# microsoft/NOTSOFAR1-Challenge

Hardware: AMD Instinct MI355X
Metric: CSS real-time-factor (sep. audio sec/wall sec) on 7-ch 16 kHz (higher is better)
Workload: dtype f32 (float32 operands on v_mfma_f32_32x32x2_f32 in every Linear layer, attention product and transform: the reference's own operand precision; MVDR covariance / solve f64)

## Files before the change

### notsofar1-challenge_amd/csrc/api_core.hip

```cpp
#include "api_ctx.hpp"

thread_local std::string g_create_error;

int fail(css_ctx* h, int code, const std::string& msg) {
    if (h) h->err = msg;
    else g_create_error = msg;
    return code;
}

int ensure(css_ctx* h, DevBuf& b, size_t bytes, bool zero) {
    if (bytes <= b.cap) return CSS_OK;
    if (b.p && h->queued) HIPCHK(h, hipDeviceSynchronize());
    if (b.p) HIPCHK(h, hipFree(b.p));
    b.p = nullptr;
    b.cap = 0;
    HIPCHK(h, hipMalloc(&b.p, bytes));
    b.cap = bytes;
    if (zero) HIPCHK(h, hipMemsetAsync(b.p, 0, bytes, h->stream));
    return CSS_OK;
}

int64_t bind_weights(const CssModelDesc& d, const float* base, Weights* w) {
    const int64_t D = d.attention_dim, FF = d.linear_units, Kp = round_up(d.in_features, 32);
    const int64_t dk = D / d.attention_heads, ks = d.kernel_size;
// ... 585 lines not shown
    if (!h || lanes < 1 || lanes > css_ctx::MAX_LANES) return fail(h, CSS_ERR_INVALID_ARG, "lanes must be in [1, 4]");
    h->lanes = lanes;
    return CSS_OK;
}

int css_get_lanes(css_handle_t h) { return h ? h->lanes : (int)CSS_ERR_INVALID_ARG; }

int css_set_tuning(css_handle_t h, int which, int value) {
    if (!h || which < 0 || which >= CSS_TUNE_COUNT || value < 0 || (value > 16 && which != CSS_TUNE_SPLIT_BATCH_ROWS && which != CSS_TUNE_F32_LANE_ROWS))
        return fail(h, CSS_ERR_INVALID_ARG, "unknown tuning option / value");
    h->tune[which] = value;
    return CSS_OK;
}

int css_set_range_fallback(css_handle_t h, int enable) {
    if (!h) return CSS_ERR_INVALID_ARG;
    h->range_fallback = enable != 0;
    return CSS_OK;
}

int css_range_status(css_handle_t h, int64_t* fallbacks, int32_t* last_hit) {
    if (!h) return CSS_ERR_INVALID_ARG;
    if (fallbacks) *fallbacks = h->range_fallbacks;
    if (last_hit) *last_hit = h->range_last;
    return CSS_OK;
}

int css_check_range(css_handle_t h) {
    int rc = check_session(h);
    if (rc) return rc;
    HIPCHK(h, hipSetDevice(h->device));
    HIPCHK(h, hipMemcpyAsync(h->range_flag_host, h->range_flag_dev, sizeof(unsigned int), hipMemcpyDeviceToHost, h->stream));
    HIPCHK(h, hipStreamSynchronize(h->stream));
    if (*h->range_flag_host && h->split)
        return fail(h, CSS_ERR_RANGE, "an operand of a Linear layer left the split-f16 range (|x| > 65504): use CSS_LINEAR_EXACT_F32");
    return CSS_OK;
}

int css_linear_host(css_handle_t h, const float* x, const float* w, const float* bias, int32_t M, int32_t N, int32_t K,
                    int32_t kernel, int32_t layout, float* y) {
    CSS_DRAIN(h);
    if (!h || !x || !w || !y || M < 1 || N < 1 || K < 32 || K % 32) return fail(h, CSS_ERR_INVALID_ARG, "bad argument (K must be a multiple of 32)");
    if (kernel < 0 || kernel > 2) return fail(h, CSS_ERR_INVALID_ARG, "kernel must be 0 (split, weights direct), 1 (split, LDS staged) or 2 (exact float32)");
    HIPCHK(h, hipSetDevice(h->device));
    const int Np = (N + 31) / 32 * 32;
    const size_t xf = (size_t)M * K, wf = (size_t)Np * K, yf = (size_t)M * N;
    int rc;
    if ((rc = ensure(h, h->stage, (2 * xf + 2 * wf + yf + (size_t)N + 256) * sizeof(float))) != CSS_OK) return rc;
    float* xd = (float*)h->stage.p;
    float* xs = xd + (xf + 15) / 16 * 16;
    float* wd = xs + (xf + 15) / 16 * 16;
    float* ws = wd + (wf + 15) / 16 * 16;
    float* yd = ws + (wf + 15) / 16 * 16;
    float* bd = yd + (yf + 15) / 16 * 16;
    HIPCHK(h, hipMemcpyAsync(xd, x, xf * sizeof(float), hipMemcpyHostToDevice, h->stream));
    HIPCHK(h, hipMemcpyAsync(wd, w, (size_t)N * K * sizeof(float), hipMemcpyHostToDevice, h->stream));
    if (bias) HIPCHK(h, hipMemcpyAsync(bd, bias, (size_t)N * sizeof(float), hipMemcpyHostToDevice, h->stream));
    GemmArgs g = linear(xd, K, wd, K, bias ? bd : nullptr, yd, N, M, N, K, ACT_NONE);
    if (kernel != 2) {
        launch_split_convert(xd, K, xs, M, K, K, h->stream);
        if (kernel == 0) launch_split_convert_tiled(wd, K, ws, N, K, h->stream);
        else launch_split_convert(wd, K, ws, N, K, K, h->stream);
        g.A = xs; g.B = ws; g.split_in = 1; g.b_tiled = kernel == 0;
        if (kernel == 0) g.tile_rows = layout; else g.layout = layout;
    } else {
        g.layout = layout;
    }
    launch_gemm(g, h->stream);
    HIPCHK(h, hipMemcpyAsync(y, yd, yf * sizeof(float), hipMemcpyDeviceToHost, h->stream));
    HIPCHK(h, hipStreamSynchronize(h->stream));
    HIPCHK(h, hipGetLastError());
    return CSS_OK;
}

int css_gemm_host(css_handle_t h, const CssGemmDesc* d, const float* a, const float* b, const float* bias, const float* residual,
                  float* c) {
    CSS_DRAIN(h);
    if (!h) return CSS_ERR_INVALID_ARG;
    auto bad = [&](const char* what) { return fail(h, CSS_ERR_INVALID_ARG, std::string("css_gemm_host: ") + what); };
    if (!d || !a || !b || !c) return bad("null argument");
    const int64_t cap = (int64_t)1 << 28;
    const int M = d->M, N = d->N, K = d->K, batch = d->batch, kernel = d->kernel;
    if (kernel < 0 || kernel > 2) return bad("kernel must be 0 (split, weights direct), 1 (split, LDS staged) or 2 (exact float32)");
    if (M < 1 || N < 1 || batch < 1 || K < 32 || K % 32 || M > (1 << 22) || N > (1 << 22) || K > (1 << 16) || batch > 1024)
        return bad("M, N, batch >= 1 and K a multiple of 32");
    if (d->lda < K || d->ldb < K || d->lda % 4 || d->ldb % 4 || d->lda > cap || d->ldb > cap) return bad("lda, ldb: multiples of 4, at least K");
    if (d->act < ACT_NONE || d->act > ACT_SIGMOID) return bad("act must be 0, 1 or 2");
    if (d->bias < 0 || d->bias > 2 || (d->bias != 0) != (bias != nullptr)) return bad("bias: 0 with NULL, 1 or 2 with an array");
    if (d->residual < 0 || d->residual > 2 || (d->residual == 1) != (residual != nullptr)) return bad("residual: 1 with an array, 0 or 2 with NULL");
    if (!(std::fabs(d->alpha) <= 3.0e38f)) return bad("alpha must be finite");
    if (d->a_off < 0 || d->c_off < 0 || d->r_off < 0 || d->a_off > 1024 || d->c_off > (1 << 20) || d->r_off > 1024) return bad("offsets");
    const bool tr = d->c_transposed != 0, has_res = d->residual != 0;
    const int rows_c = tr ? N : M, cols_c = tr ? M : N;
    if (d->ldc < cols_c || d->ldc > cap) return bad("ldc is shorter than a row of C");
    const int64_t ldr = d->residual == 2 ? d->ldc : d->ldr;
    if (d->residual == 1 && (ldr < N || ldr > cap)) return bad("ldr is shorter than a row of the residual");
    if (d->residual == 2 && batch != 1) return bad("the in-place residual takes batch 1");
    const int64_t extA = (int64_t)(M - 1) * d->lda + K, extB = (int64_t)(N - 1) * d->ldb + K;
    const int64_t extC = (int64_t)(rows_c - 1) * d->ldc + cols_c, extR = (int64_t)(M - 1) * ldr + N;
    const int64_t sA = batch > 1 ? d->strideA : 0, sB = batch > 1 ? d->strideB : 0, sC = batch > 1 ? d->strideC : 0;
    if (sA < 0 || sB < 0 || sA > cap || sB > cap || sC > cap || (sA && sA < extA) || (sB && sB < extB)) return bad("strideA, strideB: 0 or at least one matrix");
    if (batch > 1 && sC < extC) return bad("batch entries of C overlap");
    if (d->a_floats > cap || d->b_floats > cap || d->c_floats > cap || d->r_floats > cap) return bad("an array of more than 2^28 floats");
    if (d->a_floats < d->a_off + (batch - 1) * sA + extA) return bad("a is shorter than its description");
    if (d->b_floats < (batch - 1) * sB + extB) return bad("b is shorter than its description");
    if (d->c_floats < d->c_off + (batch - 1) * sC + extC) return bad("c is shorter than its description");
    if (d->residual == 1 && d->r_floats < d->r_off + extR) return bad("residual is shorter than its description");
    if (d->split_out < 0 || d->split_out % 32 || d->split_out > N || (d->split_out && kernel == 2)) return bad("split_out: a multiple of 32 up to N, kernels 0 and 1");
    if (tr && (kernel != 0 || has_res || d->split_out || d->bias == 2)) return bad("c_transposed: kernel 0, column bias and activation only");
    if (kernel == 0 && (batch != 1 || N % 32)) return bad("kernel 0 takes batch 1 and whole 32-column weight tiles");
    if (kernel == 0 && !tr && (d->c_off % 4 || d->ldc % 4)) return bad("kernel 0 writes 16-byte pieces: c_off and ldc must be multiples of 4");
    if (d->b_frag32 && (kernel != 2 || batch != 1 || N % 32)) return bad("b_frag32: kernel 2, batch 1, N a multiple of 32");
    const int lay = d->layout, tile = d->tile_rows;
    const bool lay_ok = kernel == 0 ? lay == 0
                                    : (lay == 0 || lay == 8 || lay == 4 || lay == 64 || (kernel == 2 && (lay == 1 || lay == 2 || (lay >= 11 && lay <= 14))));
    const bool tile_ok = kernel == 0 ? (tile == 0 || tile == 32 || tile == 64 || tile == 96 || tile == 128 || tile == 4 || tile == 65) : tile == 0;
    if (!lay_ok || !tile_ok) return bad("layout / tile_rows: not a tile layout of this kernel");

    HIPCHK(h, hipSetDevice(h->device));
    auto pad = [](int64_t n) { return (size_t)((n + 63) / 64 * 64); };
    const int nA = sA ? batch : 1, nB = sB ? batch : 1;
    const int Np = (N + 31) / 32 * 32;
    const size_t f_a = pad(d->a_floats), f_b = pad(d->b_floats), f_c = pad(d->c_floats), f_r = pad(d->residual == 1 ? d->r_floats : 0);
    const size_t f_as = kernel != 2 ? pad((int64_t)nA * M * K) : 0, f_bs = kernel == 0 ? pad((int64_t)Np * K) : kernel == 1 ? pad((int64_t)nB * N * K) : 0;
    const size_t f_bf = d->b_frag32 ? pad((int64_t)N * K) : 0, f_bias = pad(d->bias == 2 ? M : N);
    int rc;
    if ((rc = ensure(h, h->stage, (f_a + f_b + f_c + f_r + f_as + f_bs + f_bf + f_bias) * sizeof(float))) != CSS_OK) return rc;
    float* ad = (float*)h->stage.p;
    float* bd = ad + f_a;
    float* cd = bd + f_b;
    float* rd = cd + f_c;
    float* as = rd + f_r;
    float* bs = as + f_as;
    float* bf = bs + f_bs;
    float* biasd = bf + f_bf;
    HIPCHK(h, hipMemcpyAsync(ad, a, (size_t)d->a_floats * sizeof(float), hipMemcpyHostToDevice, h->stream));
    HIPCHK(h, hipMemcpyAsync(bd, b, (size_t)d->b_floats * sizeof(float), hipMemcpyHostToDevice, h->stream));
    HIPCHK(h, hipMemcpyAsync(cd, c, (size_t)d->c_floats * sizeof(float), hipMemcpyHostToDevice, h->stream));
    if (d->residual == 1) HIPCHK(h, hipMemcpyAsync(rd, residual, (size_t)d->r_floats * sizeof(float), hipMemcpyHostToDevice, h->stream));
    if (bias) HIPCHK(h, hipMemcpyAsync(biasd, bias, (size_t)(d->bias == 2 ? M : N) * sizeof(float), hipMemcpyHostToDevice, h->stream));

    GemmArgs g{};
    g.A = ad + d->a_off; g.lda = d->lda; g.strideA = sA;
    g.B = bd; g.ldb = d->ldb; g.strideB = sB;
    g.C = cd + d->c_off; g.ldc = d->ldc; g.strideC = sC;
    g.M = M; g.N = N; g.K = K; g.batch = batch;
    g.bias = bias ? biasd : nullptr; g.bias_along_m = d->bias == 2; g.act = d->act;
    g.residual = d->residual == 1 ? rd + d->r_off : d->residual == 2 ? g.C : nullptr;
    g.ldr = has_res ? ldr : 0; g.alpha = has_res ? d->alpha : 1.f;
    g.split_out = d->split_out; g.c_transposed = tr; g.m_fastest = d->m_fastest != 0; g.nt_store = d->nt_store != 0;
    g.concurrent = d->concurrent != 0;
    if (kernel != 2) {
        for (int z = 0; z < nA; ++z) launch_split_convert(g.A + z * sA, d->lda, as + (int64_t)z * M * K, M, K, K, h->stream);
        if (kernel == 0) launch_split_convert_tiled(bd, d->ldb, bs, N, K, h->stream);
        else for (int z = 0; z < nB; ++z) launch_split_convert(bd + z * sB, d->ldb, bs + (int64_t)z * N * K, N, K, K, h->stream);
        g.A = as; g.lda = K; g.strideA = sA ? (int64_t)M * K : 0;
        g.B = bs; g.ldb = K; g.strideB = sB ? (int64_t)N * K : 0;
        g.split_in = 1; g.b_tiled = kernel == 0;
        g.tile_rows = tile; g.layout = lay;
    } else {
        g.layout = lay;
        if (d->b_frag32) {
            launch_f32_fragments(bd, d->ldb, bf, N, K, h->stream);
            g.B = bf; g.b_frag32 = 1; g.B_rows = bd;
        }
    }
    launch_gemm(g, h->stream);
    HIPCHK(h, hipMemcpyAsync(c, cd, (size_t)d->c_floats * sizeof(float), hipMemcpyDeviceToHost, h->stream));
// ... 373 lines not shown
```

### notsofar1-challenge_amd/csrc/gemm_f32.hip

```cpp
#include <algorithm>
#include <type_traits>

#include "gemm_common.hpp"

namespace css {

namespace {

constexpr int F_BK = 16;
constexpr int F_LD = 20;
constexpr int F_BUF = (128 + BN) * F_LD;
constexpr int F_PATCH_LD = 36;

typedef float f32x4 __attribute__((ext_vector_type(4)));

__device__ __forceinline__ float epi_value(float acc, float bn, float bm, int act, bool has_res, float rv, float alpha) {
    float v = acc + bn + bm;
    if (act == ACT_RELU) v = fmaxf(v, 0.f);
    else if (act == ACT_SIGMOID) v = sigmoidf_(v);
    if (has_res) v = rv + alpha * v;
    return v;
}

template <int TM, bool BD, bool FAST>
__device__ __forceinline__ void f32_tile(const GemmArgs& g, const float* __restrict__ A, const float* __restrict__ B,
                                         float* __restrict__ C, const int m0, const int n0, float* __restrict__ lds) {
    const int tid = threadIdx.x, lane = tid & 63, w = tid >> 6, c = lane & 31, h = lane >> 5;
    const int M = g.M, N = g.N;
    constexpr int BM = 32 * TM;
    constexpr int NPA = (BM + 63) / 64;
    const int srow = tid >> 2, sk = (tid & 3) * 4;
    const int64_t extA = (int64_t)(M - 1) * g.lda + (g.lda > g.K ? g.lda : g.K), extB = (int64_t)(N - 1) * g.ldb + (g.ldb > g.K ? g.ldb : g.K);
    const __amdgpu_buffer_rsrc_t rsA = __builtin_amdgcn_make_buffer_rsrc(const_cast<float*>(A), 0, (int)(extA * 4), 0x00020000);
    const __amdgpu_buffer_rsrc_t rsB = __builtin_amdgcn_make_buffer_rsrc(const_cast<float*>(B), 0, (int)((BD ? (int64_t)((N + 31) / 32 * 32) * g.K : extB) * 4), 0x00020000);
    const int voA = (int)(((int64_t)(m0 + srow) * g.lda + sk) * 4), voB = (int)(((int64_t)(n0 + srow) * g.ldb + sk) * 4);
    const int passA = (int)(64 * g.lda * 4), passB = (int)(64 * g.ldb * 4);
    const bool a1_on = (BM % 64 == 0) || srow < BM % 64;
#ifndef F32_TOOLS
#define F32_TOOLS 0
#endif
#ifndef F32_PROBE
#define F32_PROBE 0
#endif
#ifndef F32_FAST_EPILOGUE
#define F32_FAST_EPILOGUE 1
#endif
#ifndef F32_SPREAD
#define F32_SPREAD 1
#endif
#ifndef F32_TRANSPOSED
#define F32_TRANSPOSED 0
#endif
#ifndef F32_STORE_GUARD
#define F32_STORE_GUARD 1
#endif
#if F32_STORE_GUARD
#define F32_AFTER_STORE(o) asm volatile("s_nop 0" : : "v"(o));
#else
#define F32_AFTER_STORE(o)
#endif
#ifndef F32_DMA
#define F32_DMA 0
#endif
#if F32_DMA
    constexpr int D_BUF = (128 + BN) * 16;
    const int dseg = ((tid & 3) ^ ((tid >> 4) & 3)) * 4;
    const int dvoA = (int)(((int64_t)(m0 + srow) * g.lda + dseg) * 4), dvoB = (int)(((int64_t)(n0 + srow) * g.ldb + dseg) * 4);
    const bool a1_wave = (BM % 64 == 0) || w < (BM % 64) / 16;
    typedef __attribute__((address_space(3))) void lds_void;
#define F32_GLOAD(k0, buf)                                                                                       \
    _Pragma("unroll") for (int i = 0; i < NPA; ++i) {                                                            \
        if (i + 1 < NPA || a1_wave)                                                                              \
            __builtin_amdgcn_raw_ptr_buffer_load_lds(rsA, (lds_void*)(lds + (buf) * D_BUF + (i * 64 + 16 * w) * 16), 16, dvoA, (k0) * 4 + i * passA, 0, 0); \
    }                                                                                                            \
    _Pragma("unroll") for (int i = 0; i < 2; ++i)                                                                \
        __builtin_amdgcn_raw_ptr_buffer_load_lds(rsB, (lds_void*)(lds + (buf) * D_BUF + (128 + i * 64 + 16 * w) * 16), 16, dvoB, (k0) * 4 + i * passB, 0, 0);
#define F32_LSTORE(buf) __builtin_amdgcn_s_waitcnt(0x0F70);
#define F32_GLOAD1(k0, j)
#undef F32_SPREAD
#define F32_SPREAD 0
#else
    f32x4 ra[NPA], rb[2];
    f32x4 wc[2], wn[2];
    const int vw = (int)((((int64_t)(n0 / 32 + w) * (g.K / 8)) * 64 + lane) * 16);
#define F32_GLOAD(k0, buf)                                                                                       \
    _Pragma("unroll") for (int i = 0; i < NPA; ++i) {                                                            \
        if (i + 1 < NPA || a1_on) ra[i] = __builtin_bit_cast(f32x4, __builtin_amdgcn_raw_buffer_load_b128(rsA, voA, (k0) * 4 + i * passA, 0)); \
    }                                                                                                            \
    if constexpr (!BD) {                                                                                         \
        _Pragma("unroll") for (int i = 0; i < 2; ++i)                                                            \
            rb[i] = __builtin_bit_cast(f32x4, __builtin_amdgcn_raw_buffer_load_b128(rsB, voB, (k0) * 4 + i * passB, 0)); \
    } else {                                                                                                     \
        wn[0] = __builtin_bit_cast(f32x4, __builtin_amdgcn_raw_buffer_load_b128(rsB, vw, ((k0) / 8) * 1024, 0)); \
        wn[1] = __builtin_bit_cast(f32x4, __builtin_amdgcn_raw_buffer_load_b128(rsB, vw, ((k0) / 8 + 1) * 1024, 0)); \
    }
#define F32_GLOAD1(k0, j)                                                                                        \
    {                                                                                                            \
        if ((j) < NPA) {                                                                                         \
            if ((j) + 1 < NPA || a1_on) ra[(j) < NPA ? (j) : 0] = __builtin_bit_cast(f32x4, __builtin_amdgcn_raw_buffer_load_b128(rsA, voA, (k0) * 4 + (j) * passA, 0)); \
        } else if ((j) < NPA + 2) {                                                                              \
            if constexpr (!BD) rb[(j) - NPA] = __builtin_bit_cast(f32x4, __builtin_amdgcn_raw_buffer_load_b128(rsB, voB, (k0) * 4 + ((j) - NPA) * passB, 0)); \
            else wn[(j) - NPA] = __builtin_bit_cast(f32x4, __builtin_amdgcn_raw_buffer_load_b128(rsB, vw, ((k0) / 8 + (j) - NPA) * 1024, 0)); \
        }                                                                                                        \
    }
#define F32_LSTORE(buf)                                                                                          \
    {                                                                                                            \
        float* as_ = lds + (buf) * F_BUF + srow * F_LD + sk;                                                     \
        _Pragma("unroll") for (int i = 0; i < NPA; ++i) {                                                        \
            if (i + 1 < NPA || a1_on) *reinterpret_cast<f32x4*>(as_ + i * 64 * F_LD) = ra[i];                    \
        }                                                                                                        \
        if constexpr (!BD) {                                                                                     \
            _Pragma("unroll") for (int i = 0; i < 2; ++i) *reinterpret_cast<f32x4*>(as_ + (128 + i * 64) * F_LD) = rb[i]; \
        }                                                                                                        \
    }
#endif
    f32x16 acc[TM];
#pragma unroll
    for (int i = 0; i < TM; ++i) acc[i] = f32x16{0};
    const int nk = g.K / F_BK;
#if F32_PROBE
    const unsigned long long t_in_ = (w == 0) ? __builtin_readcyclecounter() : 0;
#endif
    F32_GLOAD(0, 0)
    F32_LSTORE(0)
    if constexpr (BD) { wc[0] = wn[0]; wc[1] = wn[1]; }
    __syncthreads();
#if F32_DMA
    constexpr int S_BUF = D_BUF, S_LD = 16;
    const int sw4 = ((c >> 2) & 3) * 4;
    const int aoff = c * 16, boff = (128 + 32 * w + c) * 16;
#define F32_SLOT(ch) (((8 * (ch) + 4 * h)) ^ sw4)
#else
    constexpr int S_BUF = F_BUF, S_LD = F_LD;
    const int aoff = c * F_LD + 4 * h, boff = (128 + 32 * w + c) * F_LD + 4 * h;
#define F32_SLOT(ch) (8 * (ch))
#endif
    const float* __restrict__ bias = g.bias;
    const float* __restrict__ res = g.residual;
    const int act = g.act;
    const bool bias_m = bias && g.bias_along_m, bias_n = bias && !g.bias_along_m, has_res = res != nullptr;
    const int64_t ldc = g.ldc, ldr = g.ldr;
    const float alpha = g.alpha;
    const bool wide = FAST || ((ldc % 4 == 0) && (N % 4 == 0) && ((reinterpret_cast<uintptr_t>(C) & 15) == 0) &&
                               (!has_res || ((ldr % 4 == 0) && ((reinterpret_cast<uintptr_t>(res) & 15) == 0))));
    constexpr bool fast = FAST;
    const __amdgpu_buffer_rsrc_t rsC = __builtin_amdgcn_make_buffer_rsrc(C, 0, fast ? (int)((int64_t)M * ldc * 4) : 0, 0x00020000);
    const __amdgpu_buffer_rsrc_t rsR = __builtin_amdgcn_make_buffer_rsrc(const_cast<float*>(res), 0, (fast && has_res) ? (int)((int64_t)M * ldr * 4) : 0, 0x00020000);
    f32x4 rv[2][4];
#if F32_TRANSPOSED
    auto prefetch_fast = [&](int i, int slot, int lane_) {
        const int vo_ = (int)((((int64_t)m0 + (lane_ & 31)) * ldr + n0 + 32 * w + 4 * (lane_ >> 5)) * 4);
#pragma unroll
        for (int q = 0; q < 4; ++q)
            rv[slot][q] = __builtin_bit_cast(f32x4, __builtin_amdgcn_raw_buffer_load_b128(rsR, vo_, (int)((32 * i * ldr + 8 * q) * 4), 0));
    };
#else
    auto prefetch_fast = [&](int i, int slot, int lane_) {
        const int vo_ = (int)(((unsigned)(m0 + (lane_ >> 3)) * (unsigned)ldr + n0 + 32 * w + (lane_ & 7) * 4) * 4u);
#pragma unroll
        for (int j = 0; j < 4; ++j)
            rv[slot][j] = __builtin_bit_cast(f32x4, __builtin_amdgcn_raw_buffer_load_b128(rsR, vo_, (int)((unsigned)(32 * i + 8 * j) * (unsigned)ldr * 4u), 0));
    };
#endif
    auto prefetch = [&](int i, int slot, int lane_) {
        const int n_ = n0 + 32 * w + (lane_ & 7) * 4;
#pragma unroll
        for (int j = 0; j < 4; ++j) {
            const int m = m0 + 32 * i + (lane_ >> 3) + 8 * j;
            const int mc = m < M ? m : M - 1;
            rv[slot][j] = f32x4{0.f, 0.f, 0.f, 0.f};
            if (has_res && n_ < N) {
                if (wide) {
                    rv[slot][j] = *reinterpret_cast<const f32x4*>(res + (int64_t)mc * ldr + n_);
                } else {
#pragma unroll
                    for (int e = 0; e < 4; ++e) rv[slot][j][e] = res[(int64_t)mc * ldr + (n_ + e < N ? n_ + e : N - 1)];
                }
            }
        }
    };
#ifndef F32_ABLATE
#define F32_ABLATE 0
#endif
    f32x4 abl_a = {1.f, 2.f, 3.f, (float)lane}, abl_b = {0.5f, 0.25f, (float)w, 1.f};
#define F32_COMPUTE(buf)                                                                                         \
    {                                                                                                            \
        const float* as = lds + (buf) * S_BUF + aoff;                                                            \
        const float* bs = lds + (buf) * S_BUF + boff;                                                            \
        _Pragma("unroll") for (int ch = 0; ch < 2; ++ch) {                                                       \
            f32x4 b = abl_b;                                                                                     \
            if constexpr (BD) b = wc[ch];                                                                        \
            else if (!(F32_ABLATE & 4)) b = *reinterpret_cast<const f32x4*>(bs + F32_SLOT(ch));                  \
            f32x4 a[TM];                                                                                         \
            _Pragma("unroll") for (int i = 0; i < TM; ++i) {                                                     \
                a[i] = abl_a;                                                                                    \
                if (!(F32_ABLATE & 4)) a[i] = *reinterpret_cast<const f32x4*>(as + i * 32 * S_LD + F32_SLOT(ch)); \
            }                                                                                                    \
            __builtin_amdgcn_sched_barrier(0);                                                                   \
            _Pragma("unroll") for (int e = 0; e < 4; ++e) {                                                      \
                if (F32_SPREAD && spread_k0 >= 0 && !(e & 1)) { F32_GLOAD1(spread_k0, ch * 2 + (e >> 1)) __builtin_amdgcn_sched_barrier(0); } \
                _Pragma("unroll") for (int i = 0; i < TM; ++i) {                                                 \
                    if (F32_ABLATE & 8) asm volatile("v_mfma_f32_32x32x2_f32 %0, %1, %2, %0" : "+a"(acc[i]) : "v"(a[i][e]), "v"(b[e])); \
                    else if (F32_TRANSPOSED) acc[i] = __builtin_amdgcn_mfma_f32_32x32x2f32(b[e], a[i][e], acc[i], 0, 0, 0); \
                    else acc[i] = __builtin_amdgcn_mfma_f32_32x32x2f32(a[i][e], b[e], acc[i], 0, 0, 0);          \
                }                                                                                                \
                if (F32_SPREAD && spread_k0 >= 0) __builtin_amdgcn_sched_barrier(0);                             \
            }                                                                                                    \
            __builtin_amdgcn_sched_barrier(0);                                                                   \
        }                                                                                                        \
    }
#if F32_PROBE
    const bool probe = w == 0 && g.narrow_epilogue == 77 && g.range_flag;
    unsigned long long pc_ = 0, pl_ = 0, pb_ = 0, pt_ = 0;
    const unsigned long long t_loop_ = probe ? __builtin_readcyclecounter() : 0;
#define F32_CLK(var) if (probe) var = __builtin_readcyclecounter();
#else
#define F32_CLK(var)
#endif
    int spread_k0 = -1;
    for (int kt = 0; kt + 1 < nk; ++kt) {
#if F32_PROBE
        unsigned long long t0_ = 0, t1_ = 0, t2_ = 0, t3_ = 0;
#endif
        F32_CLK(t0_)
        if (F32_SPREAD) spread_k0 = (kt + 1) * F_BK;
        else if (!(F32_ABLATE & 2)) { F32_GLOAD((kt + 1) * F_BK, (kt + 1) & 1) }
        __builtin_amdgcn_sched_barrier(0);
        F32_COMPUTE(kt & 1)
        F32_CLK(t1_)
        if (!(F32_ABLATE & 2)) { F32_LSTORE((kt + 1) & 1) }
        if constexpr (BD) { wc[0] = wn[0]; wc[1] = wn[1]; }
        F32_CLK(t2_)
        if (!(F32_ABLATE & 1)) __syncthreads();
        F32_CLK(t3_)
#if F32_PROBE
        pc_ += t1_ - t0_; pl_ += t2_ - t1_; pb_ += t3_ - t2_; pt_ += 1;
#endif
    }
#if F32_PROBE
    if (probe && lane == 0) {
        unsigned long long* pr = reinterpret_cast<unsigned long long*>(g.range_flag) + 4096 + 4 * blockIdx.x;
        atomicAdd(pr + 0, pc_); atomicAdd(pr + 1, pl_); atomicAdd(pr + 2, pb_); atomicAdd(pr + 3, pt_);
        atomicAdd(pr + 4096 + 0, t_loop_ - t_in_);
        atomicAdd(pr + 4096 + 1, 1ull);
    }
    const unsigned long long t_out_ = probe ? __builtin_readcyclecounter() : 0;
#define F32_EPILOGUE_PROBE                                                                                       \
    if (probe && lane == 0) {                                                                                    \
        unsigned long long* pr = reinterpret_cast<unsigned long long*>(g.range_flag) + 4096 + 4 * blockIdx.x;    \
        atomicAdd(pr + 4096 + 2, __builtin_readcyclecounter() - t_out_);        \
    }
#else
#define F32_EPILOGUE_PROBE
#endif
#undef F32_CLK
    {
        int lane_ = lane;
        asm volatile("" : "+v"(lane_));
        if (fast) { if (has_res) prefetch_fast(0, 0, lane_); }
        else prefetch(0, 0, lane_);
    }
    spread_k0 = -1;
    F32_COMPUTE((nk - 1) & 1)
    __syncthreads();
#undef F32_COMPUTE
#undef F32_SLOT
#undef F32_GLOAD
#undef F32_GLOAD1
#undef F32_LSTORE

    int lane_e = lane;
    asm volatile("" : "+v"(lane_e));
    float* patch = lds + w * (32 * F_PATCH_LD);
    const int col4 = (lane_e & 7) * 4, n = n0 + 32 * w + col4, erow = lane_e >> 3;
    const bool col_ok = n < N;
    float bn[4] = {0.f, 0.f, 0.f, 0.f};
    if (bias_n) {
#pragma unroll
        for (int e = 0; e < 4; ++e) bn[e] = bias[n + e < N ? n + e : N - 1];
    }
#if F32_TRANSPOSED
    if (fast) {
        const int ce = lane_e & 31, he = lane_e >> 5, nw = n0 + 32 * w + 4 * he;
        const int voC = (int)((((int64_t)m0 + ce) * ldc + nw) * 4);
        const bool relu = act == ACT_RELU;
        f32x4 bq[4];
#pragma unroll
        for (int q = 0; q < 4; ++q) {
            bq[q] = f32x4{0.f, 0.f, 0.f, 0.f};
            if (bias_n) {
#pragma unroll
                for (int e = 0; e < 4; ++e) bq[q][e] = bias[nw + 8 * q + e];
            }
        }
#pragma unroll
        for (int i = 0; i < TM; ++i) {
            if (i + 1 < TM && has_res) prefetch_fast(i + 1, (i + 1) & 1, lane_e);
#pragma unroll
            for (int q = 0; q < 4; ++q) {
                f32x4 o;
#pragma unroll
                for (int e = 0; e < 4; ++e) {
                    float t = acc[i][4 * q + e] + bq[q][e];
                    if (relu) t = fmaxf(t, 0.f);
                    if (has_res) t = rv[i & 1][q][e] + alpha * t;
                    o[e] = t;
                }
                typedef unsigned int u32x4 __attribute__((ext_vector_type(4)));
                __builtin_amdgcn_raw_buffer_store_b128(__builtin_bit_cast(u32x4, o), rsC, voC, (int)((32 * i * ldc + 8 * q) * 4), 0);
                F32_AFTER_STORE(o)
#if F32_TRANSPOSED >= 2
                __builtin_amdgcn_sched_barrier(0);
                asm volatile("s_nop 7");
#if F32_TRANSPOSED >= 3
                asm volatile("s_nop 7");
#endif
                __builtin_amdgcn_sched_barrier(0);
#endif
            }
        }
        F32_EPILOGUE_PROBE
        return;
    }
#else
    if constexpr (FAST) {
        const int voC = (int)(((unsigned)(m0 + erow) * (unsigned)ldc + n) * 4u);
        auto epilogue = [&](auto relu_c, auto res_c) {
            const bool relu = relu_c;
            constexpr bool res = decltype(res_c)::value;
#pragma unroll
            for (int i = 0; i < TM; ++i) {
#pragma unroll
                for (int r = 0; r < 16; ++r) patch[((r & 3) + 8 * (r >> 2) + 4 * h) * F_PATCH_LD + c] = acc[i][r];
                if (i + 1 < TM && res) prefetch_fast(i + 1, (i + 1) & 1, lane_e);
#pragma unroll
                for (int j = 0; j < 4; ++j) {
                    const f32x4 v = *reinterpret_cast<const f32x4*>(patch + (erow + 8 * j) * F_PATCH_LD + col4);
                    f32x4 o;
#pragma unroll
                    for (int e = 0; e < 4; ++e) {
                        float t = v[e] + bn[e];
                        if (relu) t = fmaxf(t, 0.f);
                        if (res) t = rv[i & 1][j][e] + alpha * t;
                        o[e] = t;
                    }
                    typedef unsigned int u32x4 __attribute__((ext_vector_type(4)));
                    __builtin_amdgcn_raw_buffer_store_b128(__builtin_bit_cast(u32x4, o), rsC, voC, (int)((unsigned)(32 * i + 8 * j) * (unsigned)ldc * 4u), 0);
// ... 25 lines not shown
            const f32x4 v = *reinterpret_cast<const f32x4*>(patch + row * F_PATCH_LD + col4);
            if (m >= M || !col_ok) continue;
            float* dst = C + (int64_t)m * ldc + n;
            const float bm = bias_m ? bias[m] : 0.f;
            f32x4 o;
#pragma unroll
            for (int e = 0; e < 4; ++e) o[e] = epi_value(v[e], bn[e], bm, act, has_res, rv[i & 1][j][e], alpha);
            if (wide) {
                *reinterpret_cast<f32x4*>(dst) = o;
            } else {
#pragma unroll
                for (int e = 0; e < 4; ++e)
                    if (n + e < N) dst[e] = o[e];
            }
        }
    }
    F32_EPILOGUE_PROBE
#undef F32_EPILOGUE_PROBE
}

}

struct F32Plan {
    int u, tiles_n, ncu, max_tm; int64_t U;
#if F32_TOOLS
    unsigned long long* dbg;
#endif
};

template <bool BD, bool FAST>
__global__ __launch_bounds__(256, 4) void gemm_f32_kernel(GemmArgs g, F32Plan p) {
    __shared__ __attribute__((aligned(16))) float lds[2 * F_BUF];
    const int b = blockIdx.x, v = b % p.ncu, j = b / p.ncu;
    const int64_t lo = p.U * v / p.ncu, hi = p.U * (v + 1) / p.ncu;
    int64_t pos = lo + (hi - lo) * j / 4;
    const int64_t end = lo + (hi - lo) * (j + 1) / 4;
    int want = std::min(1 + (b + j) % 4, p.max_tm);
    bool first = true;
#if F32_TOOLS
    if (p.dbg && threadIdx.x == 0) {
        p.dbg[4 * b + 0] = wall_clock64();
        p.dbg[4 * b + 2] = ((unsigned long long)__builtin_amdgcn_s_getreg(63508) << 32) | (unsigned)__builtin_amdgcn_s_getreg(63492);
        p.dbg[4 * b + 3] = __builtin_readcyclecounter();
    }
#endif
    const int64_t panel0 = pos / p.u;
    int r = (int)(pos - panel0 * p.u);
    int bz = (int)(panel0 / p.tiles_n), tn = (int)(panel0 - (int64_t)bz * p.tiles_n);
    while (pos < end) {
        const int tm = (int)std::min<int64_t>(std::min<int64_t>(want, end - pos), p.u - r);
        const float* A = g.A + (int64_t)bz * g.strideA;
        const float* B = g.B + (int64_t)bz * g.strideB;
        float* C = g.C + (int64_t)bz * g.strideC;
        if (!first) __syncthreads();
        first = false;
        switch (tm) {
            case 1: f32_tile<1, BD, FAST>(g, A, B, C, 32 * r, tn * BN, lds); break;
            case 2: f32_tile<2, BD, FAST>(g, A, B, C, 32 * r, tn * BN, lds); break;
            case 3: f32_tile<3, BD, FAST>(g, A, B, C, 32 * r, tn * BN, lds); break;
            default: f32_tile<4, BD, FAST>(g, A, B, C, 32 * r, tn * BN, lds); break;
        }
        pos += tm;
        want = p.max_tm;
        r += tm;
        if (r == p.u) {
            r = 0;
            if (++tn == p.tiles_n) { tn = 0; ++bz; }
        }
    }
#if F32_TOOLS
    if (p.dbg && threadIdx.x == 0) { p.dbg[4 * b + 1] = wall_clock64(); p.dbg[4 * b + 3] = __builtin_readcyclecounter() - p.dbg[4 * b + 3]; }
#endif
}

static bool f32_fast_epilogue(const GemmArgs& g) {
    const int64_t lim = (int64_t)1 << 31;
    const bool has_res = g.residual != nullptr;
    const bool wide = (g.ldc % 4 == 0) && (g.N % 4 == 0) && ((reinterpret_cast<uintptr_t>(g.C) & 15) == 0) &&
                      (g.batch == 1 || g.strideC % 4 == 0) &&
                      (!has_res || ((g.ldr % 4 == 0) && ((reinterpret_cast<uintptr_t>(g.residual) & 15) == 0)));
    return F32_FAST_EPILOGUE && wide && !(g.bias && g.bias_along_m) && (g.N % BN == 0) && g.act != ACT_SIGMOID &&
           (int64_t)g.M * g.ldc * 4 < lim && (!has_res || (int64_t)g.M * g.ldr * 4 < lim);
}

bool launch_gemm_f32(const GemmArgs& g, hipStream_t s, int forced_tm) {
    if (g.M <= 0 || g.N <= 0 || g.batch <= 0) return true;
    if (g.K <= 0 || g.K % F_BK) return false;
    const int64_t lim = (int64_t)1 << 31;
    if ((((int64_t)g.M + 128) * g.lda + g.K) * 4 >= lim || (((int64_t)g.N + 128) * g.ldb + g.K) * 4 >= lim) return false;
    if (g.b_frag32 && (g.N % 32 || g.K % 16 || g.batch != 1 || ((int64_t)g.N * g.K * 4 >= lim))) return false;
    if ((g.lda % 4) || (!g.b_frag32 && (g.ldb % 4)) || (reinterpret_cast<uintptr_t>(g.A) & 15) || (reinterpret_cast<uintptr_t>(g.B) & 15)) return false;
    constexpr int NCU = 256;
    F32Plan p;
    p.u = (g.M + 31) / 32;
    p.tiles_n = (g.N + BN - 1) / BN;
    p.ncu = NCU;
    p.max_tm = (forced_tm >= 1 && forced_tm <= 4) ? forced_tm : 4;
    p.U = (int64_t)p.u * p.tiles_n * g.batch;
#if F32_TOOLS
    p.dbg = g.narrow_epilogue == 77 ? reinterpret_cast<unsigned long long*>(g.range_flag) : nullptr;
#endif
    const bool fast = f32_fast_epilogue(g);
    void (*kern)(GemmArgs, F32Plan) = g.b_frag32 ? (fast ? gemm_f32_kernel<true, true> : gemm_f32_kernel<true, false>)
                                                 : (fast ? gemm_f32_kernel<false, true> : gemm_f32_kernel<false, false>);
    hipLaunchKernelGGL(kern, dim3(4 * NCU), dim3(256), 0, s, g, p);
    return true;
}


__global__ void f32_fragments_kernel(const float* __restrict__ src, int64_t ld_src, float* __restrict__ dst, int N, int K) {
    const int64_t idx = (int64_t)blockIdx.x * blockDim.x + threadIdx.x;
    const int64_t total = (int64_t)(N / 32) * (K / 8) * 64;
    if (idx >= total) return;
    const int lane = (int)(idx & 63);
    const int64_t t = idx >> 6;
    const int kc = (int)(t % (K / 8)), j = (int)(t / (K / 8));
    const float* p = src + (int64_t)(32 * j + (lane & 31)) * ld_src + 8 * kc + 4 * (lane >> 5);
    reinterpret_cast<float4*>(dst)[idx] = make_float4(p[0], p[1], p[2], p[3]);
}
void launch_f32_fragments(const float* src, int64_t ld_src, float* dst, int N, int K, hipStream_t s) {
    const int64_t total = (int64_t)(N / 32) * (K / 8) * 64;
    if (total <= 0) return;
    hipLaunchKernelGGL(f32_fragments_kernel, dim3((unsigned)((total + 255) / 256)), dim3(256), 0, s, src, ld_src, dst, N, K);
}

}
```

### notsofar1-challenge_amd/csrc/kernels.hpp

```cpp
#pragma once
#include <hip/hip_runtime.h>
#include <stdint.h>

namespace css {

enum GemmAct : int { ACT_NONE = 0, ACT_RELU = 1, ACT_SIGMOID = 2 };

struct GemmArgs {
    const float* A; int64_t lda; int64_t strideA;
    const float* B; int64_t ldb; int64_t strideB;
    float* C; int64_t ldc; int64_t strideC;
    int M, N, K, batch;
    const float* bias;
    int bias_along_m;
    int act;
    const float* residual;
    int64_t ldr;
    float alpha;
    int split_in;
    int split_out;
    int b_tiled;
    int b_frag32;
    const float* B_rows;
    int concurrent;
    int nt_store;
    float* frag_out;
    int frag_D, frag_T, frag_heads;
    float frag_invT;
    int tile_rows;
    int narrow_epilogue;
    unsigned int* range_flag;
    int layout;
    int m_fastest;
    int c_transposed;
};
void launch_gemm(const GemmArgs& g, hipStream_t s);
bool launch_gemm_f32(const GemmArgs& g, hipStream_t s, int forced_tm);
void launch_f32_fragments(const float* src, int64_t ld_src, float* dst, int N, int K, hipStream_t s);
void launch_gemm_split(const GemmArgs& g, hipStream_t s);
void launch_gemm_split_wd(const GemmArgs& g, hipStream_t s);
void launch_split_convert_tiled(const float* src, int64_t ld_src, float* dst, int N, int K, hipStream_t s);
void launch_split_convert(const float* src, int64_t ld_src, float* dst, int64_t rows, int K, int Kp, hipStream_t s);

void launch_layernorm(const float* x, float* y, float* y_split, const float* w, const float* b, int rows, int D,
                      int relu, hipStream_t s);
void launch_layernorm2(const float* x, float* y, const float* w1, const float* b1, float* z, float* z_split,
                       const float* w2, const float* b2, int rows, int D, hipStream_t s);
void launch_ln_glu(const float* x, float* z, const float* w, const float* b, const float* pw, int rows, int D,
                   hipStream_t s);
void launch_dwconv(const float* z, float* h, const float* dw_wt, const float* dw_b, const float* bn_alpha,
                   const float* bn_beta, const float* pw, int nseg, int T, int D, int taps, hipStream_t s);
bool launch_conv_module(const float* x_in, float* x_out, const float* ln_w, const float* ln_b, const float* pw,
                        const float* dw_wt, const float* dw_b, const float* bn_alpha, const float* bn_beta,
                        const float* ln2_w, const float* ln2_b, float* z, float* z_split, int nseg, int T,
                        int D, int taps, hipStream_t s);
inline int pe_fragment_tiles(int T) { return 2 * ((T + 31) / 32); }
void launch_pe_fragments(const float* pe, float* frag, int T, int maxlen, int split, hipStream_t s);
inline int64_t qk_fragment_floats(int64_t nseg, int T, int H) { return nseg * H * ((T + 31) / 32) * 2 * 8 * 64 * 4; }
void launch_relpos_attention(const float* qkv, const float* qk_frag, const float* pe_frag, float* ctx, int nseg, int T, int D,
                             int H, int maxlen, int qk_split, int split_out, hipStream_t s);
bool launch_relpos_attention_long(const float* qkv, const float* pe, float* ctx, int nseg, int T, int D, int H, int maxlen,
                                  int split_out, hipStream_t s);

size_t stft_table_floats();
void stft_build_tables(float* host, int window = 0);
bool launch_stft_fft(const float* x, int64_t x_stride, int C, int64_t t_lo, int64_t t_hi, const float* tables, float* out,
                     int64_t row_ld, hipStream_t s, float* phase = nullptr);

__device__ __forceinline__ int css_xcd_item(int L, int n) {
    const int q = n >> 3, rem = n & 7, xcd = L & 7;
    return xcd * q + (xcd < rem ? xcd : rem) + (L >> 3);
}

#define CSS_PHASE_NEG_REAL (-3.14159250259399414f)
__device__ __forceinline__ float css_phase_of(float re, float im) {
    return (im == 0.f && re < 0.f) ? CSS_PHASE_NEG_REAL : atan2f(im, re);
}

void launch_deinterleave(const float* pcm, float* pcm_cm, int64_t n, int C, int64_t n_pad, int64_t i_lo, int64_t i_hi,
                         int split_out, hipStream_t s);
void launch_pcm_peak_f32(const float* x, int64_t count, unsigned int* peak, hipStream_t s);
void launch_pcm_peak_i16(const int16_t* x, int64_t count, unsigned int* peak, hipStream_t s);
void launch_pcm16_to_float(const int16_t* planes, float* pcm, int64_t n, int C, hipStream_t s);
void launch_pcm16_to_channel_major(const int16_t* planes, float* pcm_cm, int64_t n, int C, int64_t n_pad, int64_t i_lo,
                                   int64_t i_hi, hipStream_t s);
void launch_encode_pcm16(const float* wav, int S, int64_t n, unsigned int* peak_bits, int16_t* out, int64_t out_ld,
                         hipStream_t s);
bool css_force_long_path();

struct FeatOpts {
    int log_mag, mvn, ipd_norm, ipd_version, ipd_cos, num_pairs;
    unsigned char pair_l[16], pair_r[16];
};
void launch_features(const float* X, int64_t T_ld, int64_t stft_frames, int C, int F, float* feat, int Kp,
                     const float* in_bias, const float* in_scale, int64_t seg_lo, int nseg, int T, int hop,
                     int split_out, const FeatOpts& opts, hipStream_t s, const float* PH = nullptr);
void launch_wave_ola(const float* G, float* out, int B, int64_t T_frames, int hop, int frame_len, int64_t q_lo, int64_t q_hi,
                     int64_t f_lo, int64_t f_hi, int64_t out_ld, int64_t out_q0, const unsigned int* level, hipStream_t s);
void launch_join_shards(const float* gathered, int64_t ld, const int64_t* t_lo, const int64_t* t_hi, int world, int S, int hop,
                        int64_t n_out, float* out, int64_t out_ld, hipStream_t s);
void launch_planes_to_rows(const float* planes, float* rows, int B, int F2, int64_t T, int KIp, hipStream_t s);

void handoff_build_dft(float* m);
void handoff_build_mel(float* w, int n_mels);
void launch_handoff_gather(const float* wav, const int64_t* regions, const int64_t* offs, int nr, int64_t n_act, float* out,
                           int64_t total, hipStream_t s);
void launch_handoff_mel(const float* spec, int64_t ld, int64_t nfr, const float* w, int n_mels, float* mel, int* gmax, hipStream_t s);

constexpr int HANDOFF_TAIL_LD = 512;
constexpr int HANDOFF_GMAX_NONE = (int)0x807fffff;
struct HandoffState { int64_t A; int64_t J; int gmax; int pad_; };
struct HandoffAppend {
    const uint8_t* gate; int64_t gate_ld, gate_mask;
    const float* out; int64_t out_ld, out_base;
    const float* carry_in; float* carry_out; int64_t carry_ld;
    const float* tail_in; float* tail_out;
    const HandoffState* st;
    HandoffState* st_out;
    int64_t t_g0, t_g1, D0, D1;
    int pad, drop, closing, S;
// ... 108 lines not shown
```

Measured before the change: 7198.

## Add three-stage LDS ring for A with direct-to-LDS loads in the f32 GEMM

Adds a three-stage pipelined main loop to the persistent float32 MFMA GEMM, enabled by default when weights are pre-fragmented (BD). A slabs are loaded straight into a ring of LDS stages with buffer_load ... lds, and the loads are interleaved between MFMA groups. Vmcnt-counted waits replace the two-stage register-staged copy. The goal is to hide global load latency two slabs ahead and drop the register-to-LDS store step. The cost is hand-written inline asm that manipulates M0, tighter LDS sharing, and a relaxed host check that admits K that is a multiple of 16.

```diff
diff --git a/notsofar1-challenge_amd/csrc/api_core.hip b/notsofar1-challenge_amd/csrc/api_core.hip
--- a/notsofar1-challenge_amd/csrc/api_core.hip
+++ b/notsofar1-challenge_amd/csrc/api_core.hip
@@ -691,8 +691,10 @@
     const int64_t cap = (int64_t)1 << 28;
     const int M = d->M, N = d->N, K = d->K, batch = d->batch, kernel = d->kernel;
     if (kernel < 0 || kernel > 2) return bad("kernel must be 0 (split, weights direct), 1 (split, LDS staged) or 2 (exact float32)");
-    if (M < 1 || N < 1 || batch < 1 || K < 32 || K % 32 || M > (1 << 22) || N > (1 << 22) || K > (1 << 16) || batch > 1024)
-        return bad("M, N, batch >= 1 and K a multiple of 32");
+    const bool k16 = kernel == 2 && d->b_frag32 && (d->layout == 0 || d->layout == 1 || (d->layout >= 11 && d->layout <= 14));
+    if (M < 1 || N < 1 || batch < 1 || K < 16 || K % (k16 ? 16 : 32) || M > (1 << 22) || N > (1 << 22) || K > (1 << 16) || batch > 1024)
+        return bad("M, N, batch >= 1 and K a multiple of 32 (of 16: kernel 2 with b_frag32, layout 0, 1, 11 .. 14)");
+    if (K % 32 && (d->a_off % 4 || d->lda > (1 << 16) || d->ldb > (1 << 16))) return bad("K % 32 != 0: only what the persistent float32 kernel itself takes (a_off a multiple of 4, lda and ldb up to 65536)");
     if (d->lda < K || d->ldb < K || d->lda % 4 || d->ldb % 4 || d->lda > cap || d->ldb > cap) return bad("lda, ldb: multiples of 4, at least K");
     if (d->act < ACT_NONE || d->act > ACT_SIGMOID) return bad("act must be 0, 1 or 2");
     if (d->bias < 0 || d->bias > 2 || (d->bias != 0) != (bias != nullptr)) return bad("bias: 0 with NULL, 1 or 2 with an array");
diff --git a/notsofar1-challenge_amd/csrc/gemm_f32.hip b/notsofar1-challenge_amd/csrc/gemm_f32.hip
--- a/notsofar1-challenge_amd/csrc/gemm_f32.hip
+++ b/notsofar1-challenge_amd/csrc/gemm_f32.hip
@@ -58,6 +58,9 @@
 #define F32_AFTER_STORE(o) asm volatile("s_nop 0" : : "v"(o));
 #else
 #define F32_AFTER_STORE(o)
+#endif
+#ifndef F32_STAGES
+#define F32_STAGES 3
 #endif
 #ifndef F32_DMA
 #define F32_DMA 0
@@ -121,10 +124,13 @@
 #if F32_PROBE
     const unsigned long long t_in_ = (w == 0) ? __builtin_readcyclecounter() : 0;
 #endif
-    F32_GLOAD(0, 0)
-    F32_LSTORE(0)
-    if constexpr (BD) { wc[0] = wn[0]; wc[1] = wn[1]; }
-    __syncthreads();
+    constexpr bool RING = BD && F32_STAGES > 2;
+    if constexpr (!RING) {
+        F32_GLOAD(0, 0)
+        F32_LSTORE(0)
+        if constexpr (BD) { wc[0] = wn[0]; wc[1] = wn[1]; }
+        __syncthreads();
+    }
 #if F32_DMA
     constexpr int S_BUF = D_BUF, S_LD = 16;
     const int sw4 = ((c >> 2) & 3) * 4;
@@ -181,6 +187,12 @@
     };
 #ifndef F32_ABLATE
 #define F32_ABLATE 0
+#endif
+#if F32_STAGES != 2 && F32_STAGES != 3
+#error "F32_STAGES: 2 (two-stage loop) or 3 (A ring)"
+#endif
+#if F32_STAGES > 2 && (F32_PROBE || F32_ABLATE || F32_DMA)
+#error "F32_PROBE, F32_ABLATE and F32_DMA instrument the two-stage loop: build them with -DF32_STAGES=2"
 #endif
     f32x4 abl_a = {1.f, 2.f, 3.f, (float)lane}, abl_b = {0.5f, 0.25f, (float)w, 1.f};
 #define F32_COMPUTE(buf)                                                                                         \
@@ -217,7 +229,91 @@
 #else
 #define F32_CLK(var)
 #endif
+    if constexpr (RING) {
+        constexpr int S = F32_STAGES;
+        constexpr int R_STAGE = 128 * 64;
+        static_assert(S == 3 && S * R_STAGE <= 2 * F_BUF * 4, "the ring lives in the block's two slab buffers");
+        typedef __attribute__((address_space(3))) float lds_float;
+        const unsigned ring_0 = (unsigned)reinterpret_cast<uintptr_t>((lds_float*)lds);
+        const unsigned ring_w = ring_0 + 16 * __builtin_amdgcn_readfirstlane(w) * 64;
+        auto ring_now = [&]() { unsigned t = ring_w; asm volatile("" : "+s"(t)); return t; };
+        auto ring_a1 = [&]() { return (BM % 64 == 0) || ring_now() < ring_0 + ((BM % 64) / 16) * 16 * 64; };
+        int dvoA[NPA];
+        dvoA[0] = (int)(((int64_t)(m0 + srow) * g.lda + ((tid & 3) ^ ((tid >> 4) & 3)) * 4) * 4);
+        if constexpr (NPA == 2) dvoA[1] = dvoA[0] + passA;
+        const int rsw = ((c >> 2) & 3) * 4;
+        const float* a_ch[2] = {lds + c * 16 + ((4 * h) ^ rsw), lds + c * 16 + ((8 + 4 * h) ^ rsw)};
+#define F32_RING_A(slab, i)                                                                                      \
+    {                                                                                                            \
+        unsigned keep_;                                                                                          \
+        asm volatile("s_mov_b32 %0, m0\n\ts_mov_b32 m0, %3\n\ts_nop 4\n\tbuffer_load_dwordx4 %1, %2, %4 offen lds\n\ts_mov_b32 m0, %0" \
+                     : "=&s"(keep_)                                                                              \
+                     : "v"(dvoA[i]), "s"(rsA), "s"(ring_w + ((unsigned)(slab) % S) * R_STAGE + (i) * 64 * 64), "s"((slab) * (F_BK * 4))        \
+                     : "memory");                                                                                \
+    }
+#define F32_RING_W(slab, j) \
+    asm volatile("buffer_load_dwordx4 %0, %1, %2, %3 offen" : "=v"(wn[j]) : "v"(vw), "s"(rsB), "s"(((slab) * 2 + (j)) * 1024));
+#define F32_RING_WAIT(n) asm volatile("s_waitcnt vmcnt(%0)" : : "n"(n) : "memory");
+        auto ring_next = [&](auto behind_c, bool counted) {
+            constexpr int behind = decltype(behind_c)::value;
+            if (!counted) F32_RING_WAIT(0)
+            else if (ring_a1()) F32_RING_WAIT(behind * NPA)
+            else F32_RING_WAIT(behind * (NPA - 1))
+            asm volatile("" : "+v"(wn[0]), "+v"(wn[1]));
+            wc[0] = wn[0]; wc[1] = wn[1];
+            asm volatile("s_waitcnt lgkmcnt(0)\n\ts_barrier" : : : "memory");
+        };
+        auto ring_slab = [&](auto last_c, auto req_c, const int kt) {
+            constexpr bool last = decltype(last_c)::value, req_a = decltype(req_c)::value;
+            const int stage_f = (int)((unsigned)kt % S) * (R_STAGE / 4);
+#pragma unroll
+            for (int ch = 0; ch < 2; ++ch) {
+                const f32x4 b = wc[ch];
+                f32x4 a[TM];
+#pragma unroll
+                for (int i = 0; i < TM; ++i) a[i] = *reinterpret_cast<const f32x4*>(a_ch[ch] + stage_f + i * 32 * 16);
+                __builtin_amdgcn_sched_barrier(0);
+#pragma unroll
+                for (int e = 0; e < 4; ++e) {
+                    if (!last && !(e & 1)) {
+                        if (ch == 0) { F32_RING_W(kt + 1, e >> 1) }
+                        else if ((e >> 1) < NPA && req_a && ((e >> 1) + 1 < NPA || ring_a1())) { F32_RING_A(kt + S - 1, e >> 1) }
+                        __builtin_amdgcn_sched_barrier(0);
+                    }
+#pragma unroll
+                    for (int i = 0; i < TM; ++i) acc[i] = __builtin_amdgcn_mfma_f32_32x32x2f32(a[i][e], b[e], acc[i], 0, 0, 0);
+                    __builtin_amdgcn_sched_barrier(0);
+                }
+            }
+            if constexpr (!last) ring_next(std::integral_constant<int, 1>{}, req_a);
+        };
+        F32_RING_W(0, 0) F32_RING_W(0, 1)
+#pragma unroll
+        for (int sl = 0; sl < S - 1; ++sl) {
+            if (sl < nk) {
+#pragma unroll
+                for (int i = 0; i < NPA; ++i)
+                    if (i + 1 < NPA || ring_a1()) { F32_RING_A(sl, i) }
+            }
+        }
+        ring_next(std::integral_constant<int, S - 2>{}, nk >= S - 1);
+        int kt = 0;
+        for (; kt + S - 1 < nk; ++kt) ring_slab(std::false_type{}, std::true_type{}, kt);
+        for (; kt + 1 < nk; ++kt) ring_slab(std::false_type{}, std::false_type{}, kt);
+        {
+            int lane_ = lane;
+            asm volatile("" : "+v"(lane_));
+            if (fast) { if (has_res) prefetch_fast(0, 0, lane_); }
+            else prefetch(0, 0, lane_);
+        }
+        ring_slab(std::true_type{}, std::false_type{}, nk - 1);
+        __syncthreads();
+#undef F32_RING_A
+#undef F32_RING_W
+#undef F32_RING_WAIT
+    }
     int spread_k0 = -1;
+    if constexpr (!RING)
     for (int kt = 0; kt + 1 < nk; ++kt) {
 #if F32_PROBE
         unsigned long long t0_ = 0, t1_ = 0, t2_ = 0, t3_ = 0;
@@ -254,15 +350,17 @@
 #define F32_EPILOGUE_PROBE
 #endif
 #undef F32_CLK
-    {
-        int lane_ = lane;
-        asm volatile("" : "+v"(lane_));
-        if (fast) { if (has_res) prefetch_fast(0, 0, lane_); }
-        else prefetch(0, 0, lane_);
-    }
-    spread_k0 = -1;
-    F32_COMPUTE((nk - 1) & 1)
-    __syncthreads();
+    if constexpr (!RING) {
+        {
+            int lane_ = lane;
+            asm volatile("" : "+v"(lane_));
+            if (fast) { if (has_res) prefetch_fast(0, 0, lane_); }
+            else prefetch(0, 0, lane_);
+        }
+        spread_k0 = -1;
+        F32_COMPUTE((nk - 1) & 1)
+        __syncthreads();
+    }
 #undef F32_COMPUTE
 #undef F32_SLOT
 #undef F32_GLOAD
@@ -454,6 +552,8 @@
     return F32_FAST_EPILOGUE && wide && !(g.bias && g.bias_along_m) && (g.N % BN == 0) && g.act != ACT_SIGMOID &&
            (int64_t)g.M * g.ldc * 4 < lim && (!has_res || (int64_t)g.M * g.ldr * 4 < lim);
 }
+
+int gemm_f32_stages() { return F32_STAGES; }
 
 bool launch_gemm_f32(const GemmArgs& g, hipStream_t s, int forced_tm) {
     if (g.M <= 0 || g.N <= 0 || g.batch <= 0) return true;
diff --git a/notsofar1-challenge_amd/csrc/kernels.hpp b/notsofar1-challenge_amd/csrc/kernels.hpp
--- a/notsofar1-challenge_amd/csrc/kernels.hpp
+++ b/notsofar1-challenge_amd/csrc/kernels.hpp
@@ -36,6 +36,7 @@
 };
 void launch_gemm(const GemmArgs& g, hipStream_t s);
 bool launch_gemm_f32(const GemmArgs& g, hipStream_t s, int forced_tm);
+int gemm_f32_stages();
 void launch_f32_fragments(const float* src, int64_t ld_src, float* dst, int N, int K, hipStream_t s);
 void launch_gemm_split(const GemmArgs& g, hipStream_t s);
 void launch_gemm_split_wd(const GemmArgs& g, hipStream_t s);
```

Result: no change. 7256 (median of 6 runs) (+0.8%).
